# kyprifog/ballista

Measured on AMD Instinct MI355X. Metric: tpch_q1_sf100_rows_per_sec, higher is better.
Workload: dtype f64; 1 GPU; TPC-H Q1 SF100 (scan+filter+group-by aggregate), 600037902 lineitem rows resident in HBM, Arrow layout, Int32 order keys; lineitem_rows=600037902, rows_per_gpu=600037902, partitioning=1 GPU, whole tables

## Files before the change

### ballista_amd/_lib.py

```python
from __future__ import annotations

import ctypes as C
import os

_HERE = os.path.dirname(os.path.abspath(__file__))
LIB_PATH = os.environ.get("BHIP_LIB_PATH") or os.path.join(_HERE, "lib", "libballista_hip.so")

OK, EINVAL, ENOTIMPL, EEXEC, EHIP, EOOM = 0, 1, 2, 3, 4, 5


class BallistaError(Exception):

    def __init__(self, code, message):
        super().__init__(message)
        self.code = code


class NotImplementedOnGpu(BallistaError):
    """BHIP_ENOTIMPL — DataFusionError::NotImplemented: keep the CPU operator for this subtree."""


class PlanError(BallistaError):
    """BHIP_EINVAL — DataFusionError::Plan / Internal."""

# ... 73 lines not shown
class TpchOpts(C.Structure):
    _fields_ = [("key64", C.c_int32), ("with_dates", C.c_int32), ("sparse_keys", C.c_int32), ("n_columns", C.c_int32),
                ("key_base", C.c_int64), ("columns", C.POINTER(C.c_char_p))]


LEAF_RESOLVER = C.CFUNCTYPE(C.c_int32, C.c_void_p, C.POINTER(LeafDesc), C.POINTER(C.c_void_p))


class SortExprC(C.Structure):
    _fields_ = [("expr", Expr), ("descending", C.c_int32), ("nulls_first", C.c_int32)]


class WindowExprC(C.Structure):
    _fields_ = [("fn", C.c_int32), ("arg", Expr), ("offset", C.c_int64), ("frame", C.c_int32), ("name", C.c_char_p)]


class RowsFrameC(C.Structure):
    _fields_ = [("start_unbounded", C.c_int32), ("end_unbounded", C.c_int32), ("start", C.c_int64), ("end", C.c_int64)]


_P = C.c_void_p
_PP = C.POINTER(C.c_void_p)
SYMBOLS = {
    "bhip_last_error": (C.c_char_p, []),
    "bhip_version": (C.c_char_p, []),
    "bhip_ctx_create": (C.c_int32, [C.c_int, _PP]),
    "bhip_ctx_release": (None, [_P]),
    "bhip_ctx_synchronize": (C.c_int32, [_P]),
    "bhip_ctx_memory": (C.c_int32, [_P, C.POINTER(C.c_uint64), C.POINTER(C.c_uint64)]),
    "bhip_ctx_kernel_time": (C.c_int32, [_P, C.c_int32, C.POINTER(C.c_double), C.POINTER(C.c_uint64)]),
    "bhip_ctx_kernel_name": (C.c_char_p, [_P]),
    "bhip_ctx_kernel_variant": (C.c_char_p, [_P]),
    "bhip_ctx_lean_key_form": (C.c_char_p, [_P]),
    "bhip_ctx_sort_limit_form": (C.c_char_p, [_P]),
    "bhip_ctx_join_key_form": (C.c_char_p, [_P]),
    "bhip_ctx_nested_loop_form": (C.c_char_p, [_P]),
    "bhip_ctx_join_probe_form": (C.c_char_p, [_P]),
    "bhip_ctx_device_cus": (C.c_int32, [_P]),
    "bhip_ctx_kernel_stats": (C.c_int32, [_P, C.c_int32, C.c_char_p, C.c_size_t]),
    "bhip_batch_from_host": (C.c_int32, [_P, C.c_int32, C.POINTER(ColumnDesc), C.c_int64, _PP]),
    "bhip_batch_from_device": (C.c_int32, [_P, C.c_int32, C.POINTER(ColumnDesc), C.c_int64, _PP]),
    "bhip_batch_from_tbl": (C.c_int32, [_P, _P, C.c_int64, C.c_int32, C.POINTER(ColumnDesc), C.c_int32, C.POINTER(C.c_int32), _PP]),
    "bhip_batch_from_csv": (C.c_int32, [_P, _P, C.c_int64, C.c_int32, C.POINTER(ColumnDesc), C.c_int32, C.POINTER(C.c_int32),
                                        C.POINTER(CsvOpts), _PP]),
    "bhip_batch_import_arrow": (C.c_int32, [_P, _P, _P, _PP]),
    "bhip_batch_export_arrow": (C.c_int32, [_P, _P, _P]),
    "bhip_batch_retain": (None, [_P]),
    "bhip_batch_release": (None, [_P]),
    "bhip_batch_num_rows": (C.c_int64, [_P]),
    "bhip_batch_num_columns": (C.c_int32, [_P]),
    "bhip_batch_column_info": (C.c_int32, [_P, C.c_int32, C.POINTER(C.c_char_p), C.POINTER(C.c_int32),
                                           C.POINTER(C.c_int32), C.POINTER(C.c_int64), C.POINTER(C.c_int32)]),
    "bhip_batch_column_device": (C.c_int32, [_P, C.c_int32, _PP, _PP, _PP]),
    "bhip_batch_column_to_host": (C.c_int32, [_P, C.c_int32, _P, _P, _P]),
    "bhip_batch_memory_size": (C.c_int64, [_P]),
    "bhip_plan_memory": (C.c_int32, [_P, C.c_int32, C.POINTER(C.c_int32), _PP, _PP]),
    "bhip_plan_arrow_stream": (C.c_int32, [_P, _P, _PP]),
    "bhip_plan_arrow_streams": (C.c_int32, [_P, C.c_int32, _PP, _PP]),
    "bhip_plan_parquet": (C.c_int32, [_P, C.c_int32, C.POINTER(C.c_char_p), C.c_int32, C.POINTER(C.c_uint32), C.c_int32, _PP]),
    "bhip_plan_text_scan": (C.c_int32, [_P, C.c_int32, C.POINTER(C.c_char_p), C.c_int32, C.POINTER(ColumnDesc), C.c_int32,
                                        C.POINTER(C.c_int32), C.POINTER(TextScanOpts), _PP]),
    "bhip_plan_empty": (C.c_int32, [_P, C.c_int32, C.POINTER(ColumnDesc), C.c_int32, _PP]),
    "bhip_plan_filter": (C.c_int32, [_P, C.POINTER(Expr), _PP]),
    "bhip_plan_projection": (C.c_int32, [_P, C.c_int32, C.POINTER(Expr), C.POINTER(C.c_char_p), _PP]),
    "bhip_plan_hash_aggregate": (C.c_int32, [_P, C.c_int32, C.c_int32, C.POINTER(Expr), C.POINTER(C.c_char_p),
                                             C.c_int32, C.POINTER(Aggregate), _PP]),
# ... 81 lines not shown
```

### ballista_amd/csrc/host/capi.cpp

```cpp
#include <cstdio>
#include <cstring>

#include "../util_kernels.h"
#include "plan.hpp"

using namespace bhip;

#define BHIP_API_BEGIN try {
#define BHIP_API_END                                              \
    return BHIP_OK;                                               \
    }                                                             \
    catch (const bhip::Error& e) {                                \
        bhip::set_last_error(e.what());                           \
        return e.code;                                            \
    }                                                             \
    catch (const std::bad_alloc&) {                               \
        bhip::set_last_error("host allocation failed");           \
        return BHIP_EOOM;                                         \
    }                                                             \
    catch (const std::exception& e) {                             \
        bhip::set_last_error(std::string("internal error: ") + e.what()); \
        return BHIP_EINVAL;                                       \
    }                                                             \
    catch (...) {                                                 \
// ... 50 lines not shown
    need(ctx, "ctx"); need(buf, "buf");
    ctx->p->set_device();
    std::string text;
    for (auto& kv : ctx->p->kernel_stats(reset != 0)) {
        char line[256];
        snprintf(line, sizeof line, "%s\t%.6f\t%llu\t%llu\n", kv.first.c_str(), kv.second.ms, (unsigned long long)kv.second.launches,
                 (unsigned long long)kv.second.bytes);
        text += line;
    }
    if (text.size() + 1 > cap) fail(BHIP_EINVAL, "bhip_ctx_kernel_stats: buffer too small");
    memcpy(buf, text.c_str(), text.size() + 1);
    BHIP_API_END
}

const char* bhip_ctx_kernel_name(bhip_ctx* ctx) {
    static thread_local std::string name;
    name = ctx ? ctx->p->kernel_name() : std::string();
    return name.c_str();
}

int32_t bhip_ctx_device_cus(bhip_ctx* ctx) {
    return ctx ? ctx->p->cus() : 0;
}

const char* bhip_ctx_kernel_variant(bhip_ctx* ctx) {
    static thread_local std::string name;
    name = ctx ? ctx->p->kernel_variant() : std::string();
    return name.c_str();
}

const char* bhip_ctx_lean_key_form(bhip_ctx* ctx) {
    static thread_local std::string name;
    name = ctx ? ctx->p->lean_key_form() : std::string();
    return name.c_str();
}

const char* bhip_ctx_sort_limit_form(bhip_ctx* ctx) {
    static thread_local std::string name;
    name = ctx ? ctx->p->sort_limit_form() : std::string();
    return name.c_str();
}

const char* bhip_ctx_join_key_form(bhip_ctx* ctx) {
    static thread_local std::string name;
    name = ctx ? ctx->p->join_key_form() : std::string();
    return name.c_str();
}

const char* bhip_ctx_nested_loop_form(bhip_ctx* ctx) {
    static thread_local std::string name;
    name = ctx ? ctx->p->nested_loop_form() : std::string();
    return name.c_str();
}

const char* bhip_ctx_join_probe_form(bhip_ctx* ctx) {
    static thread_local std::string name;
    name = ctx ? ctx->p->join_probe_form() : std::string();
    return name.c_str();
}

static bhip_batch* wrap_batch(BatchPtr b) {
    auto h = new bhip_batch();
    h->p = std::move(b);
    return h;
}

// ... 654 lines not shown
```

### ballista_amd/csrc/host/core.cpp

```cpp
#include "core.hpp"

#include <immintrin.h>

#include <chrono>
#include <cstdlib>

#include "../util_kernels.h"

__attribute__((constructor)) static void bhip_runtime_defaults() { setenv("HIP_FORCE_DEV_KERNARG", "1", 0); }

namespace bhip {

static thread_local std::string t_last_error;
void set_last_error(const std::string& m) { t_last_error = m; }
const char* get_last_error() { return t_last_error.c_str(); }

const char* dtype_name(int dt) {
    switch (dt) {
        case DT_INT32: return "Int32";
        case DT_INT64: return "Int64";
        case DT_UINT8: return "UInt8";
        case DT_UINT64: return "UInt64";
        case DT_FLOAT64: return "Float64";
        case DT_DATE32: return "Date32";
// ... 251 lines not shown
        if (hipEventSynchronize(p.b) == hipSuccess && hipEventElapsedTime(&t, p.a, p.b) == hipSuccess) {
            auto& st = k_stats_[p.name];
            st.ms += t;
            st.launches += 1;
            st.bytes += p.bytes;
        }
        event_pool_.push_back(p.a);
        event_pool_.push_back(p.b);
    }
    pending_timed_.clear();
    auto out = k_stats_;
    if (reset) k_stats_.clear();
    return out;
}

std::string Context::kernel_name() {
    std::lock_guard<std::mutex> g(mu_);
    return k_name_;
}

std::string Context::kernel_variant() {
    std::lock_guard<std::mutex> g(mu_);
    return k_variant_;
}

void Context::set_lean_key_form(const char* form) {
    std::lock_guard<std::mutex> g(mu_);
    k_key_form_ = form ? form : "";
}

std::string Context::lean_key_form() {
    std::lock_guard<std::mutex> g(mu_);
    return k_key_form_;
}

void Context::set_sort_limit_form(const char* form) {
    std::lock_guard<std::mutex> g(mu_);
    k_sort_limit_form_ = form ? form : "";
}

std::string Context::sort_limit_form() {
    std::lock_guard<std::mutex> g(mu_);
    return k_sort_limit_form_;
}

void Context::set_join_key_form(const char* form) {
    std::lock_guard<std::mutex> g(mu_);
    k_join_key_form_ = form ? form : "";
}

std::string Context::join_key_form() {
    std::lock_guard<std::mutex> g(mu_);
    return k_join_key_form_;
}

void Context::set_nested_loop_form(const char* form) {
    std::lock_guard<std::mutex> g(mu_);
    k_nested_loop_form_ = form ? form : "";
}

std::string Context::nested_loop_form() {
    std::lock_guard<std::mutex> g(mu_);
    return k_nested_loop_form_;
}

void Context::set_join_probe_form(const char* form) {
// ... 189 lines not shown
```

### ballista_amd/csrc/host/core.hpp

```cpp
#pragma once
#include <hip/hip_runtime.h>
#include <atomic>
#include <cstdint>
#include <cstring>
#include <map>
#include <memory>
#include <mutex>
#include <stdexcept>
#include <string>
#include <vector>

#include "../../../include/ballista_hip.h"
#include "../kernels.h"

namespace bhip {

struct Error : std::runtime_error {
    bhip_status code;
    Error(bhip_status c, const std::string& m) : std::runtime_error(m), code(c) {}
};
[[noreturn]] inline void fail(bhip_status c, const std::string& m) { throw Error(c, m); }
inline void hip_check(hipError_t e, const char* what) {
    if (e != hipSuccess) {
        if (e == hipErrorOutOfMemory) fail(BHIP_EOOM, std::string(what) + ": " + hipGetErrorString(e));
// ... 10 lines not shown

class Context;

struct Block {
    void* ptr = nullptr;
    size_t bytes = 0;
    hipStream_t last_stream = nullptr;
    hipEvent_t ready = nullptr;
};

class Context : public std::enable_shared_from_this<Context> {
public:
    explicit Context(int device);
    ~Context();
    int device() const { return device_; }
    int cus() const { return cus_; }
    void set_device() const { HIP_CHECK(hipSetDevice(device_)); }

    void* alloc(size_t bytes, hipStream_t stream);
    void free(void* ptr, hipStream_t stream);
    void memory(uint64_t* in_use, uint64_t* peak);
    void trim();

    hipStream_t acquire_stream();
    void release_stream(hipStream_t s);

    void wait_stream(hipStream_t stream, const void* dev_src = nullptr, void* host_dst = nullptr, size_t bytes = 0);

    void add_kernel_time(double ms, uint64_t launches, const char* kernel = nullptr, const char* variant = nullptr);
    std::string kernel_name();
    std::string kernel_variant();
    void set_lean_key_form(const char* form);
    std::string lean_key_form();
    void set_sort_limit_form(const char* form);
    std::string sort_limit_form();
    void set_join_key_form(const char* form);
    std::string join_key_form();
    void set_nested_loop_form(const char* form);
    std::string nested_loop_form();
    void set_join_probe_form(const char* form);
    std::string join_probe_form();
    void kernel_time(bool reset, double* ms, uint64_t* launches);
    bool timing_enabled() const { return timing_ > 0; }
    int timing_level() const { return timing_; }
    struct KernelStat { double ms = 0; uint64_t launches = 0; uint64_t bytes = 0; };
    void push_timed(hipEvent_t a, hipEvent_t b, const char* name, uint64_t bytes = 0);
    hipEvent_t timing_event();
    std::map<std::string, KernelStat> kernel_stats(bool reset);

private:
    int device_;
    int cus_ = 256;
    int timing_ = 0;
    std::mutex mu_;
    std::multimap<size_t, Block> free_blocks_;
    std::map<void*, Block> live_;
    uint64_t in_use_ = 0, peak_ = 0, cached_ = 0;
    std::vector<hipStream_t> stream_pool_;
    static constexpr size_t N_SLOTS = 1024;
    struct HostSlot { volatile uint64_t w[8]; };
    HostSlot* slots_ = nullptr;
    std::atomic<uint64_t> slot_seq_{0};
    bool spin_wait_ = true;
    double k_ms_ = 0;
    uint64_t k_launches_ = 0;
    std::string k_name_, k_variant_, k_key_form_, k_sort_limit_form_, k_join_key_form_, k_nested_loop_form_, k_join_probe_form_;
    struct PendingTimed { hipEvent_t a, b; const char* name; uint64_t bytes; };
    std::vector<PendingTimed> pending_timed_;
    std::vector<hipEvent_t> event_pool_;
    std::map<std::string, KernelStat> k_stats_;
};
using ContextPtr = std::shared_ptr<Context>;

struct Exec {
    ContextPtr ctx;
    hipStream_t stream;
    LaunchCfg cfg() const { return LaunchCfg{ctx->cus(), stream}; }
};

struct KernelTimer {
    const Exec& ex;
    const char* name;
    hipEvent_t a = nullptr, b = nullptr;
    uint64_t bytes = 0;
    KernelTimer(const Exec& e, const char* n, int64_t rows = -1, uint64_t algorithmic_bytes = 0) : ex(e), name(n), bytes(algorithmic_bytes) {
        const int level = ex.ctx->timing_level();
        if (level <= 0 || (level == 1 && rows < (1 << 18))) return;
        a = ex.ctx->timing_event();
        b = ex.ctx->timing_event();
        hipEventRecord(a, ex.stream);
    }
    void stop() {
        if (!a) return;
        hipEventRecord(b, ex.stream);
        ex.ctx->push_timed(a, b, name, bytes);
        a = b = nullptr;
    }
    ~KernelTimer() { stop(); }
};
// ... 168 lines not shown
```

### ballista_amd/csrc/host/ops_agg.cpp

```cpp
#include "../sort_kernels.h"
#include "../util_kernels.h"
#include "hash_kernels.h"
#include "plan.hpp"
#include "sop.hpp"

namespace bhip {

static int sum_type(int t) {
    if (dt_is_float(t)) return t;
    if (dt_is_unsigned(t)) return DT_UINT64;
    return DT_INT64;
}

static int minmax_kind(int t, bool is_min) {
    if (dt_is_float(t)) return is_min ? ACC_MIN_F64 : ACC_MAX_F64;
    if (dt_is_unsigned(t)) return is_min ? ACC_MIN_U64 : ACC_MAX_U64;
    return is_min ? ACC_MIN_I64 : ACC_MAX_I64;
}

static const char* lowcard_launch_name(int gmax, bool batches) {
    if (batches) return gmax == 1 ? "scan_agg_lowcard_g1_batches" : gmax == 4 ? "scan_agg_lowcard_g4_batches" : "scan_agg_lowcard_g8_batches";
    return gmax == 1 ? "scan_agg_lowcard_g1" : gmax == 4 ? "scan_agg_lowcard_g4" : "scan_agg_lowcard_g8";
}

// ... 477 lines not shown
        HIP_CHECK(hipMemsetAsync(status, 0, sizeof(ScanStatus), ex.stream));
        int n_part = 0;
        const bool lean_now = use_lean && (gmax == 1 || gmax == 4);
        const bool sop_now = !lean_now && use_sop;
        key_layout = lean_now || sop_now ? &sop.key_info : &pb.key_info();
        int64_t cur_rows = 0;
        for (auto& b : cur) cur_rows += b->n_rows;
        const bool together = !lean_now && !sop_now && cur.size() > 1 && cur.size() <= 4096 && cur_rows <= (1 << 20);
        bool lens_seen = lean_now && !sampling;
        std::vector<ScanParams> Ps;
        if (together) {
            Ps.assign(cur.size(), P0);
            for (size_t i = 0; i < cur.size(); ++i) ProgramBuilder::bind(Ps[i], pb.columns(), *cur[i], nullable);
            int grid = 0;
            TIMED_LAUNCH(ex, lowcard_launch_name(gmax, true),
                         launch_scan_agg_lowcard(cfg, Ps[0], tmp.get<ScanParams>(cur.size()), gmax, partials, partial_ng, max_grid, status, &grid, (int)cur.size()));
            n_part = grid;
        }
        for (auto& b : cur) {
            if (together) break;
            ScanParams P = P0;
            ProgramBuilder::bind(P, pb.columns(), *b, nullable);
            int grid = 0;
            const bool timed = b->n_rows >= (1 << 16) || ((lean_now || sop_now) && ex.ctx->timing_level() >= 2);
            if (timed) {
                timer.begin();
                timer.kernel = lean_now ? "scan_agg_lean_kernel" : sop_now ? "scan_agg_sop_kernel" : "scan_agg_lowcard_kernel";
                timer.variant = nullptr;
            }
            if (lean_now) {
                bind_sop(sop, *b);
                const char* variant = nullptr;
                bool fixed_keys = false;
                HIP_CHECK(launch_scan_agg_lean(cfg, sop.prog, tmp.get<SopProgram>(1), gmax, partials + (size_t)n_part * gmax,
                                               partial_ng + n_part, max_grid, status, &grid, &variant, &fixed_keys));
                if (timed) timer.variant = variant;
                bool utf8_key = false;
                for (int q = 0; q < sop.prog.n_keys; ++q) utf8_key = utf8_key || sop.prog.keys[q].kind == SOP_KEY_UTF8;
                ex.ctx->set_lean_key_form(fixed_keys ? "fixed" : utf8_key ? "offsets" : "none");
                lens_seen = lens_seen && !fixed_keys;
            } else if (sop_now) {
                bind_sop(sop, *b);
                HIP_CHECK(launch_scan_agg_sop(cfg, sop.prog, tmp.get<SopProgram>(1), gmax, partials + (size_t)n_part * gmax,
                                              partial_ng + n_part, max_grid, status, &grid));
            } else
                TIMED_LAUNCH(ex, lowcard_launch_name(gmax, false),
                             launch_scan_agg_lowcard(cfg, P, tmp.get<ScanParams>(1), gmax, partials + (size_t)n_part * gmax,
                                                     partial_ng + n_part, max_grid, status, &grid));
            if (timed) timer.end();
            n_part += grid;
        }
        const int cap = 1024;
        table = tmp.get<GroupRec>(cap);
        uint32_t* entry_group = tmp.get<uint32_t>((size_t)n_part * gmax);
        AccSpec specs[VM_MAX_ACC];
        for (int i = 0; i < n_acc; ++i) specs[i] = P0.acc[i];
        TIMED_LAUNCH(ex, "merge_partials", launch_merge_partials(cfg, partials, partial_ng, n_part, gmax, specs, n_acc, table, cap, entry_group, status));
        early = EmitColumns();
        if (!sampling && !no_early_emit && group_.size() <= (size_t)TAIL_TOTALS) early = emit_table(table, cap, status, *key_layout);
        trace_point("aggregate: scan + merge + emit queued");
        tail = read_device(ex, info);
        const ScanStatus st = tail.st;
        timer.collect();
        if (lean_now && (st.flags & SCAN_ERR_KEY_TOO_LONG)) {
            use_lean = false;
            continue;
        }
        if (sop_now && (st.flags & SCAN_ERR_KEY_TOO_LONG)) {
            use_sop = false;
            continue;
        }
        check_scan_flags(st);
// ... 68 lines not shown
```

### ballista_amd/csrc/kernels_lean_spec.hip

```cpp
#include <stdlib.h>
#include "lean_spec_kernel.h"

namespace bhip {

hipError_t launch_scan_agg_lean_spec(const LaunchCfg& cfg, const SopProgram& S, SopProgram* dprog, int gmax, GroupRec* partials,
                                     uint32_t* partial_ng, int max_grid, ScanStatus* status, int* grid_out, bool* ran,
                                     const char** variant, bool* fixed) {
    static const bool no_fixed = env_flag("BHIP_NO_FIXED_UTF8");
#define BHIP_LEAN_SPEC(NAME_, GMAX_, NR_, R32_, K0_, K1_, NS_)                                                            \
    if (gmax == GMAX_ && !(no_fixed && (K0_ == LK_UTF8_FIXED || K1_ == LK_UTF8_FIXED)) &&                                 \
        lean_shape_matches<NR_, R32_, K0_, K1_, NS_>(S)) {                                                                \
        *ran = true;                                                                                                      \
        *variant = NAME_;                                                                                                 \
        *fixed = K0_ == LK_UTF8_FIXED || K1_ == LK_UTF8_FIXED;                                                            \
        return launch_sop_program(scan_agg_lean_spec_kernel<GMAX_, NR_, R32_, K0_, K1_, NS_>, LEAN_TILE, cfg, S, dprog,   \
                                  partials, partial_ng, max_grid, status, grid_out);                                      \
    }
    BHIP_LEAN_SPEC("lean_spec_q1", 4, 1, 0b1, LK_UTF8_FIXED, LK_UTF8_FIXED, 5)
    BHIP_LEAN_SPEC("lean_spec_q1", 4, 1, 0b1, LK_UTF8, LK_UTF8, 5)
    BHIP_LEAN_SPEC("lean_spec_key1", 4, 1, 0b1, LK_UTF8_FIXED, LK_NONE, 5)
    BHIP_LEAN_SPEC("lean_spec_key1", 4, 1, 0b1, LK_UTF8, LK_NONE, 5)
#undef BHIP_LEAN_SPEC
    *ran = false;
    return hipSuccess;
}

}
```

### ballista_amd/csrc/kernels_sop.hip

```cpp
#include <hip/hip_runtime.h>
#include <stdlib.h>
#include "sop.h"

namespace bhip {

hipError_t launch_scan_agg_sop_g1(const LaunchCfg&, const SopProgram&, SopProgram*, GroupRec*, uint32_t*, int, ScanStatus*, int*);
hipError_t launch_scan_agg_sop_g4(const LaunchCfg&, const SopProgram&, SopProgram*, GroupRec*, uint32_t*, int, ScanStatus*, int*);
hipError_t launch_scan_agg_sop_g8(const LaunchCfg&, const SopProgram&, SopProgram*, GroupRec*, uint32_t*, int, ScanStatus*, int*);

hipError_t launch_scan_agg_sop(const LaunchCfg& cfg, const SopProgram& S, SopProgram* dprog, int gmax, GroupRec* partials,
                               uint32_t* partial_ng, int max_grid, ScanStatus* status, int* grid_out) {
    switch (gmax) {
        case 1: return launch_scan_agg_sop_g1(cfg, S, dprog, partials, partial_ng, max_grid, status, grid_out);
        case 4: return launch_scan_agg_sop_g4(cfg, S, dprog, partials, partial_ng, max_grid, status, grid_out);
        case 8: return launch_scan_agg_sop_g8(cfg, S, dprog, partials, partial_ng, max_grid, status, grid_out);
        default: return hipErrorInvalidValue;
    }
}

hipError_t launch_scan_agg_lean_g1(const LaunchCfg&, const SopProgram&, SopProgram*, GroupRec*, uint32_t*, int, ScanStatus*, int*);
hipError_t launch_scan_agg_lean_g4(const LaunchCfg&, const SopProgram&, SopProgram*, GroupRec*, uint32_t*, int, ScanStatus*, int*);
hipError_t launch_scan_agg_lean_spec(const LaunchCfg&, const SopProgram&, SopProgram*, int, GroupRec*, uint32_t*, int, ScanStatus*, int*,
                                     bool*, const char**, bool*);

hipError_t launch_scan_agg_lean(const LaunchCfg& cfg, const SopProgram& S, SopProgram* dprog, int gmax, GroupRec* partials,
                                uint32_t* partial_ng, int max_grid, ScanStatus* status, int* grid_out, const char** variant,
                                bool* fixed_keys) {
    static const bool generic_only = env_flag("BHIP_LEAN_GENERIC");
    const char* name = "lean_generic";
    bool fixed = false;
    if (!variant) variant = &name;
    if (!fixed_keys) fixed_keys = &fixed;
    *fixed_keys = false;
    if (!generic_only) {
        bool ran = false;
        const hipError_t e = launch_scan_agg_lean_spec(cfg, S, dprog, gmax, partials, partial_ng, max_grid, status, grid_out, &ran, variant, fixed_keys);
        if (ran || e != hipSuccess) return e;
    }
    *variant = "lean_generic";
    switch (gmax) {
        case 1: return launch_scan_agg_lean_g1(cfg, S, dprog, partials, partial_ng, max_grid, status, grid_out);
        case 4: return launch_scan_agg_lean_g4(cfg, S, dprog, partials, partial_ng, max_grid, status, grid_out);
        default: return hipErrorInvalidValue;
    }
}

}
```

### ballista_amd/csrc/lean_spec_kernel.h

```cpp
#pragma once
#include "lean_kernel.h"

namespace bhip {

enum LeanKeyKind : int { LK_NONE = 0, LK_I32 = 1, LK_UTF8 = 2, LK_UTF8_FIXED = 3 };

template <int GMAX, int NR, int R32, int K0, int K1, int NS>
__global__ void __launch_bounds__(BLOCK, (GMAX == 1 && NS <= 5) ? 4 : 3)
scan_agg_lean_spec_kernel(const SopProgram* __restrict__ Sp, GroupRec* partials, uint32_t* partial_ng, ScanStatus* status) {
    static_assert(NR >= 1 && NR <= SOP_NRANGE && NS >= 1 && NS <= SOP_NSTEP && (K0 != LK_NONE || K1 == LK_NONE), "lean shape");
    const SopProgram& S = *Sp;
    constexpr int U = LEAN_U;
    constexpr int NKEY = 2;
    constexpr int KK[NKEY] = {K0, K1};
    constexpr bool HAS_OFFSETS = K0 == LK_UTF8 || K1 == LK_UTF8;
    constexpr bool HAS_FIXED = K0 == LK_UTF8_FIXED || K1 == LK_UTF8_FIXED;
    static_assert(!(HAS_OFFSETS && HAS_FIXED), "no mixed key forms: one unknown width sends the plan to the offsets form");
    __shared__ LeanLds<GMAX, NS> lds;
    const int tid = threadIdx.x, lane = tid & 63;

    const int64_t n_rows = S.n_rows;
    const int64_t n_tiles = n_rows / LEAN_TILE;
    const int64_t grid = gridDim.x;
    const int64_t my_tiles = (int64_t)blockIdx.x < n_tiles ? (n_tiles - 1 - (int64_t)blockIdx.x) / grid + 1 : 0;

    const BHIP_GLOBAL char* rbase[NR];
    double rlo[NR], rhi[NR];
#pragma unroll
    for (int p = 0; p < NR; ++p) {
        rbase[p] = (const BHIP_GLOBAL char*)S.cols[S.ranges[p].col].data;
        rlo[p] = S.ranges[p].lo; rhi[p] = S.ranges[p].hi;
    }
    const BHIP_GLOBAL char* kbase[NKEY];
    const BHIP_GLOBAL char* kdat[NKEY];
    uint32_t kw[NKEY];
#pragma unroll
    for (int q = 0; q < NKEY; ++q) {
        kbase[q] = nullptr; kdat[q] = nullptr; kw[q] = 0;
        if (KK[q] != LK_NONE) {
            const SopColumn c = S.cols[S.keys[q].col];
            kbase[q] = KK[q] == LK_UTF8 ? (const BHIP_GLOBAL char*)c.offsets : (const BHIP_GLOBAL char*)c.data;
            kdat[q] = (const BHIP_GLOBAL char*)c.data;
            if (KK[q] == LK_UTF8_FIXED) {
// ... 49 lines not shown
        }
    };
    auto add_row = [&](int lgr) {
        if constexpr (GMAX == 1) {
            rows1 += lgr >= 0 ? 1u : 0u;
        } else {
            const int g = lgr >= 0 ? lgr : 0;
            __hip_atomic_fetch_add(&lds.cnt[g * BLOCK + tid], lgr >= 0 ? 1u : 0u, __ATOMIC_RELAXED, __HIP_MEMORY_SCOPE_WORKGROUP);
        }
    };

    LeanU4 rv[NR][U];
    uint32_t kv[NKEY][U][2];
    uint64_t kb[NKEY][U];
    LeanU3 ko[2][NKEY][U];
    LeanU4 xv[NS][U];
#pragma unroll
    for (int u = 0; u < U; ++u) {
#pragma unroll
        for (int p = 0; p < NR; ++p) rv[p][u] = LeanU4{0, 0, 0, 0};
#pragma unroll
        for (int q = 0; q < NKEY; ++q) {
            kv[q][u][0] = kv[q][u][1] = 0; kb[q][u] = 0;
            ko[0][q][u] = ko[1][q][u] = LeanU3{0, 0, 0};
        }
    }
    const uint32_t t8 = (uint32_t)tid * 8u, t16 = (uint32_t)tid * 16u;
    uint32_t t2w[NKEY];
#pragma unroll
    for (int q = 0; q < NKEY; ++q) t2w[q] = (uint32_t)tid * 2u * kw[q];

    auto load_step = [&](int s, int64_t row) {
#pragma unroll
        for (int u = 0; u < U; ++u) xv[s][u] = lean_ld4(xbase[s] + (row + u * LEAN_SUB) * 8 + t16);
    };
    auto load_ranges = [&](int64_t row) {
#pragma unroll
        for (int p = 0; p < NR; ++p) {
            if ((R32 >> p) & 1) {
#pragma unroll
                for (int u = 0; u < U; ++u) {
                    const LeanU2 v = lean_ld2(rbase[p] + (row + u * LEAN_SUB) * 4 + t8);
                    rv[p][u].x = v.x; rv[p][u].y = v.y;
                }
            } else {
#pragma unroll
                for (int u = 0; u < U; ++u) rv[p][u] = lean_ld4(rbase[p] + (row + u * LEAN_SUB) * 8 + t16);
            }
        }
    };
    auto load_int_keys = [&](int64_t row) {
#pragma unroll
        for (int q = 0; q < NKEY; ++q)
            if (KK[q] == LK_I32) {
#pragma unroll
                for (int u = 0; u < U; ++u) {
                    const LeanU2 v = lean_ld2(kbase[q] + (row + u * LEAN_SUB) * 4 + t8);
                    kv[q][u][0] = v.x; kv[q][u][1] = v.y;
                }
            }
    };
    auto load_offsets = [&](LeanU3 (&o)[NKEY][U], int64_t row) {
#pragma unroll
        for (int q = 0; q < NKEY; ++q)
            if (KK[q] == LK_UTF8) {
#pragma unroll
                for (int u = 0; u < U; ++u) {
                    const BHIP_GLOBAL char* a = kbase[q] + (row + u * LEAN_SUB) * 4 + t8;
                    const LeanU2 v = lean_ld2(a);
                    o[q][u].a = v.x; o[q][u].b = v.y;
                    o[q][u].c = *(const BHIP_GLOBAL uint32_t*)(a + 8);
                }
            }
    };
    auto load_key_bytes = [&](const LeanU3 (&o)[NKEY][U]) {
#pragma unroll
        for (int q = 0; q < NKEY; ++q)
            if (KK[q] == LK_UTF8) {
#pragma unroll
                for (int u = 0; u < U; ++u) {
                    const uint32_t l0 = o[q][u].b - o[q][u].a, l1 = o[q][u].c - o[q][u].b;
                    lens.see(q, l0); lens.see(q, l1);
                    kv[q][u][0] = l0; kv[q][u][1] = l1;
                    kb[q][u] = ((const BHIP_GLOBAL PackedU64*)(kdat[q] + o[q][u].a))->v;
                }
            }
    };

    auto load_key_bytes_fixed = [&](int64_t row) {
#pragma unroll
// ... 43 lines not shown
                }
            } else if (KK[q] == LK_UTF8_FIXED) {
#pragma unroll
                for (int u = 0; u < U; ++u) {
                    w[q][2 * u] = lean_str_word((uint32_t)kb[q][u], kw[q]);
                    w[q][2 * u + 1] = lean_str_word((uint32_t)(kb[q][u] >> (kw[q] << 3)), kw[q]);
                }
            } else if (KK[q] == LK_I32) {
#pragma unroll
                for (int u = 0; u < U; ++u) { w[q][2 * u] = kv[q][u][0]; w[q][2 * u + 1] = kv[q][u][1]; }
            }
        }
#pragma unroll
        for (int r = 0; r < LEAN_ROWS; ++r) key[r] = ((uint64_t)w[1][r] << 32) | w[0][r];
    };
    auto tile = [&](auto P_, auto NEXT_, int64_t k) -> bool {
        constexpr int P = decltype(P_)::value;
        constexpr bool NEXT = decltype(NEXT_)::value;
        const int64_t row1 = tile_row(k + 1);
        bool live[LEAN_ROWS];
        uint64_t key[LEAN_ROWS];
        eval_live(live);
        eval_keys(key);
        if constexpr (NEXT) {
            load_ranges(row1);
            load_int_keys(row1);
            load_key_bytes(ko[P ^ 1]);
            load_key_bytes_fixed(row1);
            if constexpr (HAS_OFFSETS) load_offsets(ko[P], tile_row(k + 2));
        }
        int lg[LEAN_ROWS];
        if (!lookup(key, live, lg)) return false;
        double tp[LEAN_ROWS];
#pragma unroll
        for (int s = 0; s < NS; ++s) {
            double tv[LEAN_ROWS];
#pragma unroll
            for (int u = 0; u < U; ++u) {
                const LeanU4 x = xv[s][u];
                double a = u2d(((uint64_t)x.y << 32) | x.x), b = u2d(((uint64_t)x.w << 32) | x.z);
                if (!xplain[s]) {
                    a = u2d(((uint64_t)(x.y ^ xflip[s]) << 32) | x.x) + xadd[s];
                    b = u2d(((uint64_t)(x.w ^ xflip[s]) << 32) | x.z) + xadd[s];
                }
                tv[2 * u] = a; tv[2 * u + 1] = b;
            }
            if (s > 0 && !xstart[s]) {
#pragma unroll
                for (int r = 0; r < LEAN_ROWS; ++r) tv[r] = tp[r] * tv[r];
            }
#pragma unroll
            for (int r = 0; r < LEAN_ROWS; ++r) { add_step(lg[r], s, tv[r]); tp[r] = tv[r]; }
            if constexpr (NEXT) load_step(s, row1);
        }
#pragma unroll
        for (int r = 0; r < LEAN_ROWS; ++r) add_row(lg[r]);
        return true;
    };
    using I0 = std::integral_constant<int, 0>;
    using I1 = std::integral_constant<int, 1>;
    using BT = std::integral_constant<bool, true>;
    using BF = std::integral_constant<bool, false>;

    bool over = false;
    if (my_tiles > 0) {
        const int64_t row0 = tile_row(0);
        if constexpr (HAS_OFFSETS) load_offsets(ko[0], row0);
        load_key_bytes(ko[0]);
        load_key_bytes_fixed(row0);
        load_ranges(row0);
        load_int_keys(row0);
        if constexpr (HAS_OFFSETS) load_offsets(ko[1], tile_row(1));
#pragma unroll
        for (int s = 0; s < NS; ++s) load_step(s, row0);
        __builtin_amdgcn_s_waitcnt(0x0F70);
        int64_t k = 0;
        for (; k + 2 < my_tiles; k += 2) {
            if (!tile(I0{}, BT{}, k) || !tile(I1{}, BT{}, k + 1)) { over = true; break; }
        }
        if (!over) {
            if (my_tiles - k == 2) over = !tile(I0{}, BT{}, k) || !tile(I1{}, BF{}, k + 1);
            else over = !tile(I0{}, BF{}, k);
        }
    }

    if (!over && (int64_t)blockIdx.x == n_tiles % grid && n_tiles * LEAN_TILE < n_rows) {
        auto accumulate = [&](int lgr, const double (&tv)[NS]) {
#pragma unroll
            for (int s = 0; s < NS; ++s) add_step(lgr, s, tv[s]);
            add_row(lgr);
        };
        LeanLens<(GMAX > 1)> tail_lens;
        over = !lean_tail<GMAX, NS, NR>(S, n_tiles * LEAN_TILE, n_rows, HAS_FIXED ? tail_lens : lens, lookup, accumulate);
    }
    lean_finish<GMAX, NS>(lds, S, acc, rows1, lens, partials, partial_ng, status);
}

template <int NR, int R32, int K0, int K1, int NS>
static bool lean_shape_matches(const SopProgram& S) {
    if (S.n_ranges != NR || S.n_steps != NS) return false;
    for (int p = 0; p < NR; ++p) {
        if ((S.ranges[p].is32 != 0) != (((R32 >> p) & 1) != 0)) return false;
        if (S.cols[S.ranges[p].col].validity) return false;
    }
    const int kk[2] = {K0, K1};
    int n_keys = 0;
    for (int q = 0; q < 2; ++q) {
        if (kk[q] == LK_NONE) continue;
        ++n_keys;
        if (S.n_keys <= q) return false;
        if (S.keys[q].kind != (kk[q] == LK_I32 ? SOP_KEY_I32 : SOP_KEY_UTF8)) return false;
        const int32_t w = S.cols[S.keys[q].col].width;
        if (kk[q] == LK_UTF8_FIXED && (w < 1 || w > (int32_t)LEAN_MAX_STR)) return false;
    }
    return S.n_keys == n_keys;
}

}
```

### ballista_amd/csrc/sop.h

```cpp
#pragma once
#include <hip/hip_runtime.h>
#include <stdint.h>
#include "kernels.h"

namespace bhip {

constexpr int SOP_NRANGE = 4;
constexpr int SOP_NKEY = 3;
constexpr int SOP_NSTEP = 8;
constexpr int SOP_NCOL = 16;

struct SopColumn {
    const void* data;
    const int32_t* offsets;
    const uint64_t* validity;
    int32_t dtype;
    int32_t data_bytes;
    int32_t width;
    int32_t pad;
};

struct SopRange {
    uint8_t col;
    uint8_t is32;
// ... 2 lines not shown
};

struct SopStep {
    uint8_t col;
    uint8_t is32;
    uint8_t has_col;
    uint8_t start;
    uint8_t acc;
    uint8_t pad[3];
    double sgn, add;
};

enum SopKeyKind : uint8_t { SOP_KEY_I32 = 0, SOP_KEY_I64 = 1, SOP_KEY_UTF8 = 2 };
struct SopKey {
    uint8_t col;
    uint8_t kind;
    uint8_t pad[2];
};

struct SopProgram {
    int64_t n_rows;
    int32_t n_cols, n_ranges, n_keys, n_steps;
    SopColumn cols[SOP_NCOL];
    SopRange ranges[SOP_NRANGE];
    SopKey keys[SOP_NKEY];
    SopStep steps[SOP_NSTEP];
};

hipError_t launch_scan_agg_sop(const LaunchCfg& cfg, const SopProgram& S, SopProgram* dprog, int gmax, GroupRec* partials,
                               uint32_t* partial_ng, int max_grid, ScanStatus* status, int* grid_out);

hipError_t launch_scan_agg_lean(const LaunchCfg& cfg, const SopProgram& S, SopProgram* dprog, int gmax, GroupRec* partials,
                                uint32_t* partial_ng, int max_grid, ScanStatus* status, int* grid_out, const char** variant = nullptr,
                                bool* fixed_keys = nullptr);

hipError_t launch_range_bitmap(const LaunchCfg& cfg, const SopProgram& S, SopProgram* dprog, uint64_t* bitmap, uint32_t* tile_counts);
struct Utf8Literal { uint8_t bytes[64]; int32_t len; };
hipError_t launch_utf8_eq_bitmap(const LaunchCfg& cfg, const int32_t* offsets, const void* data, const uint64_t* validity, int64_t n, const Utf8Literal& lit,
                                 bool negate, uint64_t* bitmap, uint32_t* tile_counts);

}
```

### ballista_amd/plan.py

```python
from __future__ import annotations

import ctypes as C
import os
from typing import Iterator, List, Optional, Sequence, Tuple

import numpy as np

from . import _lib as L
from . import expr as E

DTYPE_ID = {E.INT32: 1, E.INT64: 2, E.UINT8: 3, E.UINT64: 4, E.FLOAT64: 5, E.DATE32: 6, E.BOOLEAN: 7, E.UTF8: 8,
            "Int8": 9, "Int16": 10, "UInt16": 11, "UInt32": 12, "Float32": 13, "Date64": 14, "Timestamp(Second)": 15,
            "Timestamp(Millisecond)": 16, "Timestamp(Microsecond)": 17, "Timestamp(Nanosecond)": 18,
            "LargeUtf8": 19, "Binary": 20}
DTYPE_NAME = {v: k for k, v in DTYPE_ID.items()}
NP_DTYPE = {E.INT32: np.int32, E.INT64: np.int64, E.UINT8: np.uint8, E.UINT64: np.uint64,
            E.FLOAT64: np.float64, E.DATE32: np.int32, E.INT8: np.int8, E.INT16: np.int16, E.UINT16: np.uint16,
            E.UINT32: np.uint32, E.FLOAT32: np.float32, E.DATE64: np.int64, E.TIMESTAMP_S: np.int64,
            E.TIMESTAMP_MS: np.int64, E.TIMESTAMP_US: np.int64, E.TIMESTAMP_NS: np.int64}

PARTIAL, FINAL = "Partial", "Final"
SINGLE = "Single"
INNER, LEFT, RIGHT = "Inner", "Left", "Right"
FULL, SEMI, ANTI, RIGHT_SEMI, RIGHT_ANTI = "Full", "Semi", "Anti", "RightSemi", "RightAnti"
# ... 18 lines not shown
        return {0: "UnknownPartitioning", 1: "RoundRobinBatch", 2: "Hash"}[self.scheme] + f"({self.count})"


class Context:

    def __init__(self, device: int = 0):
        h = C.c_void_p()
        L.check(L.lib().bhip_ctx_create(device, C.byref(h)))
        self._h = h

    def synchronize(self):
        L.check(L.lib().bhip_ctx_synchronize(self._h))

    def memory(self):
        a, b = C.c_uint64(), C.c_uint64()
        L.check(L.lib().bhip_ctx_memory(self._h, C.byref(a), C.byref(b)))
        return a.value, b.value

    def kernel_time(self, reset=False):
        ms, n = C.c_double(), C.c_uint64()
        L.check(L.lib().bhip_ctx_kernel_time(self._h, 1 if reset else 0, C.byref(ms), C.byref(n)))
        return ms.value, n.value

    def kernel_name(self, variant=False):
        name = L.lib().bhip_ctx_kernel_name(self._h).decode()
        if variant:
            v = L.lib().bhip_ctx_kernel_variant(self._h).decode()
            if v:
                name += "/" + v
        return name

    def lean_key_form(self):
        return L.lib().bhip_ctx_lean_key_form(self._h).decode()

    def sort_limit_form(self):
        return L.lib().bhip_ctx_sort_limit_form(self._h).decode()

    def join_key_form(self):
        return L.lib().bhip_ctx_join_key_form(self._h).decode()

    def join_probe_form(self):
        return L.lib().bhip_ctx_join_probe_form(self._h).decode()

    def nested_loop_form(self):
        return L.lib().bhip_ctx_nested_loop_form(self._h).decode()

    def device_cus(self):
        return int(L.lib().bhip_ctx_device_cus(self._h))

    def kernel_stats(self, reset=False):
        buf = C.create_string_buffer(1 << 16)
        L.check(L.lib().bhip_ctx_kernel_stats(self._h, 1 if reset else 0, buf, len(buf)))
        out = {}
        for line in buf.value.decode().splitlines():
            name, ms, n, nbytes = line.split("\t")
            out[name] = (float(ms), int(n), int(nbytes))
        return out

    def __del__(self):
        try:
            if getattr(self, "_h", None):
                L.lib().bhip_ctx_release(self._h)
                self._h = None
        except Exception:
            pass

# ... 1018 lines not shown
```

### include/ballista_hip.h

```cpp
#ifndef BALLISTA_HIP_H
#define BALLISTA_HIP_H

#include <stddef.h>
#include <stdint.h>

#ifdef __cplusplus
extern "C" {
#endif

#ifndef ARROW_C_DATA_INTERFACE
#define ARROW_C_DATA_INTERFACE
#define ARROW_FLAG_DICTIONARY_ORDERED 1
#define ARROW_FLAG_NULLABLE 2
#define ARROW_FLAG_MAP_KEYS_SORTED 4
struct ArrowSchema {
    const char* format;
    const char* name;
    const char* metadata;
    int64_t flags;
    int64_t n_children;
    struct ArrowSchema** children;
    struct ArrowSchema* dictionary;
    void (*release)(struct ArrowSchema*);
    void* private_data;
// ... 294 lines not shown
    uint64_t rows_in, rows_out, chunks, streamed;
    uint64_t bytes_sent_remote, bytes_kept_local, staging_bytes;
    uint64_t rows_to[BHIP_SHUFFLE_MAX_PEERS];
    double ms_count, ms_total;
} bhip_shuffle_stats;
bhip_status bhip_comm_shuffle(bhip_comm* comm, bhip_batch* batch, const char* key_column, int64_t chunk_rows, bhip_batch** out,
                              bhip_shuffle_stats* stats);
bhip_status bhip_plan_all_gather(bhip_comm* comm, bhip_plan* input, bhip_plan** out);
bhip_status bhip_plan_shuffle(bhip_comm* comm, bhip_plan* input, const char* key_column, int64_t chunk_rows, bhip_plan** out);
bhip_status bhip_batch_pack(bhip_batch* batch, int64_t* header, int32_t header_cap, void* host_block, int64_t block_cap,
                            int64_t* block_bytes);
bhip_status bhip_batch_unpack(bhip_ctx* ctx, int32_t n_cols, const bhip_column_desc* schema, const int64_t* header,
                              const void* host_block, bhip_batch** out);

bhip_status bhip_tpch_lineitem(bhip_ctx* ctx, double sf, uint64_t seed, uint64_t row0, uint64_t n, int32_t key64,
                               int32_t with_dates, bhip_batch** out);
bhip_status bhip_tpch_orders(bhip_ctx* ctx, double sf, uint64_t seed, uint64_t row0, uint64_t n, int32_t key64,
                             bhip_batch** out);
typedef struct bhip_tpch_opts {
    int32_t key64, with_dates, sparse_keys, n_columns;
    int64_t key_base;
    const char* const* columns;
} bhip_tpch_opts;
bhip_status bhip_tpch_lineitem_opts(bhip_ctx* ctx, double sf, uint64_t seed, uint64_t row0, uint64_t n, const bhip_tpch_opts* opts,
                                    bhip_batch** out);
bhip_status bhip_tpch_orders_opts(bhip_ctx* ctx, double sf, uint64_t seed, uint64_t row0, uint64_t n, const bhip_tpch_opts* opts,
                                  bhip_batch** out);

bhip_status bhip_ctx_kernel_time(bhip_ctx* ctx, int32_t reset, double* ms, uint64_t* launches);
bhip_status bhip_ctx_kernel_stats(bhip_ctx* ctx, int32_t reset, char* buf, size_t cap);
const char* bhip_ctx_kernel_name(bhip_ctx* ctx);
const char* bhip_ctx_kernel_variant(bhip_ctx* ctx);
const char* bhip_ctx_lean_key_form(bhip_ctx* ctx);
const char* bhip_ctx_sort_limit_form(bhip_ctx* ctx);
const char* bhip_ctx_join_key_form(bhip_ctx* ctx);
const char* bhip_ctx_nested_loop_form(bhip_ctx* ctx);
const char* bhip_ctx_join_probe_form(bhip_ctx* ctx);
int32_t bhip_ctx_device_cus(bhip_ctx* ctx);

#ifdef __cplusplus
}
#endif
#endif
```

Before: 157.7 billion rows/s.

## Alias repeated column loads in lean Q1 kernel and use nontemporal streaming loads

Detects aggregation steps that read the same input column (Q1's sum(l_quantity), avg(l_quantity) and similar repeats, alias pattern 0,1,2,3,2) and specializes the lean kernel so each distinct column is loaded once and its value reused for the aliased steps. Separately, the column, range and key loads switch to nontemporal loads so streamed data does not pollute the cache. This targets redundant HBM traffic in a bandwidth-bound scan. It doubles the number of template instantiations and adds a diagnostic API for reporting the alias map.

```diff
diff --git a/ballista_amd/_lib.py b/ballista_amd/_lib.py
--- a/ballista_amd/_lib.py
+++ b/ballista_amd/_lib.py
@@ -129,6 +129,7 @@
     "bhip_ctx_kernel_name": (C.c_char_p, [_P]),
     "bhip_ctx_kernel_variant": (C.c_char_p, [_P]),
     "bhip_ctx_lean_key_form": (C.c_char_p, [_P]),
+    "bhip_ctx_lean_step_alias": (C.c_char_p, [_P]),
     "bhip_ctx_sort_limit_form": (C.c_char_p, [_P]),
     "bhip_ctx_join_key_form": (C.c_char_p, [_P]),
     "bhip_ctx_nested_loop_form": (C.c_char_p, [_P]),
diff --git a/ballista_amd/csrc/host/capi.cpp b/ballista_amd/csrc/host/capi.cpp
--- a/ballista_amd/csrc/host/capi.cpp
+++ b/ballista_amd/csrc/host/capi.cpp
@@ -106,6 +106,12 @@
 const char* bhip_ctx_lean_key_form(bhip_ctx* ctx) {
     static thread_local std::string name;
     name = ctx ? ctx->p->lean_key_form() : std::string();
+    return name.c_str();
+}
+
+const char* bhip_ctx_lean_step_alias(bhip_ctx* ctx) {
+    static thread_local std::string name;
+    name = ctx ? ctx->p->lean_step_alias() : std::string();
     return name.c_str();
 }
 
diff --git a/ballista_amd/csrc/host/core.cpp b/ballista_amd/csrc/host/core.cpp
--- a/ballista_amd/csrc/host/core.cpp
+++ b/ballista_amd/csrc/host/core.cpp
@@ -307,6 +307,23 @@
 std::string Context::lean_key_form() {
     std::lock_guard<std::mutex> g(mu_);
     return k_key_form_;
+}
+
+void Context::set_lean_step_alias(uint32_t alias, int n_steps) {
+    std::string list;
+    bool aliased = false;
+    for (int s = 0; s < n_steps; ++s) {
+        const int a = (int)((alias >> (4 * s)) & 15u);
+        aliased = aliased || a != s;
+        list += (s ? "," : "") + std::to_string(a);
+    }
+    std::lock_guard<std::mutex> g(mu_);
+    k_step_alias_ = aliased ? list : "none";
+}
+
+std::string Context::lean_step_alias() {
+    std::lock_guard<std::mutex> g(mu_);
+    return k_step_alias_;
 }
 
 void Context::set_sort_limit_form(const char* form) {
diff --git a/ballista_amd/csrc/host/core.hpp b/ballista_amd/csrc/host/core.hpp
--- a/ballista_amd/csrc/host/core.hpp
+++ b/ballista_amd/csrc/host/core.hpp
@@ -66,6 +66,8 @@
     std::string kernel_variant();
     void set_lean_key_form(const char* form);
     std::string lean_key_form();
+    void set_lean_step_alias(uint32_t alias, int n_steps);
+    std::string lean_step_alias();
     void set_sort_limit_form(const char* form);
     std::string sort_limit_form();
     void set_join_key_form(const char* form);
@@ -98,7 +100,7 @@
     bool spin_wait_ = true;
     double k_ms_ = 0;
     uint64_t k_launches_ = 0;
-    std::string k_name_, k_variant_, k_key_form_, k_sort_limit_form_, k_join_key_form_, k_nested_loop_form_, k_join_probe_form_;
+    std::string k_name_, k_variant_, k_key_form_, k_step_alias_, k_sort_limit_form_, k_join_key_form_, k_nested_loop_form_, k_join_probe_form_;
     struct PendingTimed { hipEvent_t a, b; const char* name; uint64_t bytes; };
     std::vector<PendingTimed> pending_timed_;
     std::vector<hipEvent_t> event_pool_;
diff --git a/ballista_amd/csrc/host/ops_agg.cpp b/ballista_amd/csrc/host/ops_agg.cpp
--- a/ballista_amd/csrc/host/ops_agg.cpp
+++ b/ballista_amd/csrc/host/ops_agg.cpp
@@ -533,12 +533,14 @@
                 bind_sop(sop, *b);
                 const char* variant = nullptr;
                 bool fixed_keys = false;
+                uint32_t step_alias = 0;
                 HIP_CHECK(launch_scan_agg_lean(cfg, sop.prog, tmp.get<SopProgram>(1), gmax, partials + (size_t)n_part * gmax,
-                                               partial_ng + n_part, max_grid, status, &grid, &variant, &fixed_keys));
+                                               partial_ng + n_part, max_grid, status, &grid, &variant, &fixed_keys, &step_alias));
                 if (timed) timer.variant = variant;
                 bool utf8_key = false;
                 for (int q = 0; q < sop.prog.n_keys; ++q) utf8_key = utf8_key || sop.prog.keys[q].kind == SOP_KEY_UTF8;
                 ex.ctx->set_lean_key_form(fixed_keys ? "fixed" : utf8_key ? "offsets" : "none");
+                ex.ctx->set_lean_step_alias(step_alias, sop.prog.n_steps);
                 lens_seen = lens_seen && !fixed_keys;
             } else if (sop_now) {
                 bind_sop(sop, *b);
diff --git a/ballista_amd/csrc/kernels_lean_spec.hip b/ballista_amd/csrc/kernels_lean_spec.hip
--- a/ballista_amd/csrc/kernels_lean_spec.hip
+++ b/ballista_amd/csrc/kernels_lean_spec.hip
@@ -5,22 +5,30 @@
 
 hipError_t launch_scan_agg_lean_spec(const LaunchCfg& cfg, const SopProgram& S, SopProgram* dprog, int gmax, GroupRec* partials,
                                      uint32_t* partial_ng, int max_grid, ScanStatus* status, int* grid_out, bool* ran,
-                                     const char** variant, bool* fixed) {
+                                     const char** variant, bool* fixed, uint32_t* step_alias) {
     static const bool no_fixed = env_flag("BHIP_NO_FIXED_UTF8");
-#define BHIP_LEAN_SPEC(NAME_, GMAX_, NR_, R32_, K0_, K1_, NS_)                                                            \
+    static const bool no_alias = env_flag("BHIP_LEAN_NO_ALIAS");
+    const uint32_t alias = lean_step_alias(S);
+#define BHIP_LEAN_SPEC_A(NAME_, GMAX_, NR_, R32_, K0_, K1_, NS_, ALIAS_)                                                  \
     if (gmax == GMAX_ && !(no_fixed && (K0_ == LK_UTF8_FIXED || K1_ == LK_UTF8_FIXED)) &&                                 \
+        (ALIAS_ == lean_alias_identity(NS_) || (!no_alias && alias == ALIAS_)) &&                                         \
         lean_shape_matches<NR_, R32_, K0_, K1_, NS_>(S)) {                                                                \
         *ran = true;                                                                                                      \
         *variant = NAME_;                                                                                                 \
         *fixed = K0_ == LK_UTF8_FIXED || K1_ == LK_UTF8_FIXED;                                                            \
-        return launch_sop_program(scan_agg_lean_spec_kernel<GMAX_, NR_, R32_, K0_, K1_, NS_>, LEAN_TILE, cfg, S, dprog,   \
-                                  partials, partial_ng, max_grid, status, grid_out);                                      \
+        *step_alias = ALIAS_;                                                                                             \
+        return launch_sop_program(scan_agg_lean_spec_kernel<GMAX_, NR_, R32_, K0_, K1_, NS_, ALIAS_>, LEAN_TILE, cfg, S,  \
+                                  dprog, partials, partial_ng, max_grid, status, grid_out);                               \
     }
+#define BHIP_LEAN_SPEC(NAME_, GMAX_, NR_, R32_, K0_, K1_, NS_)                                                            \
+    BHIP_LEAN_SPEC_A(NAME_, GMAX_, NR_, R32_, K0_, K1_, NS_, 0x23210u)                                                    \
+    BHIP_LEAN_SPEC_A(NAME_, GMAX_, NR_, R32_, K0_, K1_, NS_, lean_alias_identity(NS_))
     BHIP_LEAN_SPEC("lean_spec_q1", 4, 1, 0b1, LK_UTF8_FIXED, LK_UTF8_FIXED, 5)
     BHIP_LEAN_SPEC("lean_spec_q1", 4, 1, 0b1, LK_UTF8, LK_UTF8, 5)
     BHIP_LEAN_SPEC("lean_spec_key1", 4, 1, 0b1, LK_UTF8_FIXED, LK_NONE, 5)
     BHIP_LEAN_SPEC("lean_spec_key1", 4, 1, 0b1, LK_UTF8, LK_NONE, 5)
 #undef BHIP_LEAN_SPEC
+#undef BHIP_LEAN_SPEC_A
     *ran = false;
     return hipSuccess;
 }
diff --git a/ballista_amd/csrc/kernels_sop.hip b/ballista_amd/csrc/kernels_sop.hip
--- a/ballista_amd/csrc/kernels_sop.hip
+++ b/ballista_amd/csrc/kernels_sop.hip
@@ -21,23 +21,27 @@
 hipError_t launch_scan_agg_lean_g1(const LaunchCfg&, const SopProgram&, SopProgram*, GroupRec*, uint32_t*, int, ScanStatus*, int*);
 hipError_t launch_scan_agg_lean_g4(const LaunchCfg&, const SopProgram&, SopProgram*, GroupRec*, uint32_t*, int, ScanStatus*, int*);
 hipError_t launch_scan_agg_lean_spec(const LaunchCfg&, const SopProgram&, SopProgram*, int, GroupRec*, uint32_t*, int, ScanStatus*, int*,
-                                     bool*, const char**, bool*);
+                                     bool*, const char**, bool*, uint32_t*);
 
 hipError_t launch_scan_agg_lean(const LaunchCfg& cfg, const SopProgram& S, SopProgram* dprog, int gmax, GroupRec* partials,
                                 uint32_t* partial_ng, int max_grid, ScanStatus* status, int* grid_out, const char** variant,
-                                bool* fixed_keys) {
+                                bool* fixed_keys, uint32_t* step_alias) {
     static const bool generic_only = env_flag("BHIP_LEAN_GENERIC");
     const char* name = "lean_generic";
     bool fixed = false;
+    uint32_t alias = 0;
     if (!variant) variant = &name;
     if (!fixed_keys) fixed_keys = &fixed;
+    if (!step_alias) step_alias = &alias;
     *fixed_keys = false;
     if (!generic_only) {
         bool ran = false;
-        const hipError_t e = launch_scan_agg_lean_spec(cfg, S, dprog, gmax, partials, partial_ng, max_grid, status, grid_out, &ran, variant, fixed_keys);
+        const hipError_t e = launch_scan_agg_lean_spec(cfg, S, dprog, gmax, partials, partial_ng, max_grid, status, grid_out, &ran, variant, fixed_keys, step_alias);
         if (ran || e != hipSuccess) return e;
     }
     *variant = "lean_generic";
+    *step_alias = 0;
+    for (int s = 0; s < S.n_steps; ++s) *step_alias |= (uint32_t)s << (4 * s);
     switch (gmax) {
         case 1: return launch_scan_agg_lean_g1(cfg, S, dprog, partials, partial_ng, max_grid, status, grid_out);
         case 4: return launch_scan_agg_lean_g4(cfg, S, dprog, partials, partial_ng, max_grid, status, grid_out);
diff --git a/ballista_amd/csrc/lean_spec_kernel.h b/ballista_amd/csrc/lean_spec_kernel.h
--- a/ballista_amd/csrc/lean_spec_kernel.h
+++ b/ballista_amd/csrc/lean_spec_kernel.h
@@ -5,10 +5,36 @@
 
 enum LeanKeyKind : int { LK_NONE = 0, LK_I32 = 1, LK_UTF8 = 2, LK_UTF8_FIXED = 3 };
 
-template <int GMAX, int NR, int R32, int K0, int K1, int NS>
+constexpr uint32_t lean_alias_of(uint32_t alias, int s) { return (alias >> (4 * s)) & 15u; }
+constexpr uint32_t lean_alias_identity(int ns) {
+    uint32_t a = 0;
+    for (int s = 0; s < ns; ++s) a |= (uint32_t)s << (4 * s);
+    return a;
+}
+constexpr bool lean_alias_valid(uint32_t alias, int ns) {
+    for (int s = 0; s < ns; ++s) {
+        const uint32_t a = lean_alias_of(alias, s);
+        if (a > (uint32_t)s || lean_alias_of(alias, (int)a) != a) return false;
+    }
+    return true;
+}
+
+typedef uint32_t LeanV2 __attribute__((ext_vector_type(2)));
+typedef uint32_t LeanV4 __attribute__((ext_vector_type(4)));
+__device__ inline LeanU2 lean_stream_ld2(const BHIP_GLOBAL char* p) {
+    const LeanV2 v = __builtin_nontemporal_load((const BHIP_GLOBAL LeanV2*)p);
+    return LeanU2{v.x, v.y};
+}
+__device__ inline LeanU4 lean_stream_ld4(const BHIP_GLOBAL char* p) {
+    const LeanV4 v = __builtin_nontemporal_load((const BHIP_GLOBAL LeanV4*)p);
+    return LeanU4{v.x, v.y, v.z, v.w};
+}
+
+template <int GMAX, int NR, int R32, int K0, int K1, int NS, uint32_t ALIAS = lean_alias_identity(NS)>
 __global__ void __launch_bounds__(BLOCK, (GMAX == 1 && NS <= 5) ? 4 : 3)
 scan_agg_lean_spec_kernel(const SopProgram* __restrict__ Sp, GroupRec* partials, uint32_t* partial_ng, ScanStatus* status) {
     static_assert(NR >= 1 && NR <= SOP_NRANGE && NS >= 1 && NS <= SOP_NSTEP && (K0 != LK_NONE || K1 == LK_NONE), "lean shape");
+    static_assert(lean_alias_valid(ALIAS, NS), "a(s) <= s and a(a(s)) == a(s)");
     const SopProgram& S = *Sp;
     constexpr int U = LEAN_U;
     constexpr int NKEY = 2;
@@ -124,7 +150,7 @@
 
     auto load_step = [&](int s, int64_t row) {
 #pragma unroll
-        for (int u = 0; u < U; ++u) xv[s][u] = lean_ld4(xbase[s] + (row + u * LEAN_SUB) * 8 + t16);
+        for (int u = 0; u < U; ++u) xv[s][u] = lean_stream_ld4(xbase[s] + (row + u * LEAN_SUB) * 8 + t16);
     };
     auto load_ranges = [&](int64_t row) {
 #pragma unroll
@@ -132,12 +158,12 @@
             if ((R32 >> p) & 1) {
 #pragma unroll
                 for (int u = 0; u < U; ++u) {
-                    const LeanU2 v = lean_ld2(rbase[p] + (row + u * LEAN_SUB) * 4 + t8);
+                    const LeanU2 v = lean_stream_ld2(rbase[p] + (row + u * LEAN_SUB) * 4 + t8);
                     rv[p][u].x = v.x; rv[p][u].y = v.y;
                 }
             } else {
 #pragma unroll
-                for (int u = 0; u < U; ++u) rv[p][u] = lean_ld4(rbase[p] + (row + u * LEAN_SUB) * 8 + t16);
+                for (int u = 0; u < U; ++u) rv[p][u] = lean_stream_ld4(rbase[p] + (row + u * LEAN_SUB) * 8 + t16);
             }
         }
     };
@@ -147,7 +173,7 @@
             if (KK[q] == LK_I32) {
 #pragma unroll
                 for (int u = 0; u < U; ++u) {
-                    const LeanU2 v = lean_ld2(kbase[q] + (row + u * LEAN_SUB) * 4 + t8);
+                    const LeanU2 v = lean_stream_ld2(kbase[q] + (row + u * LEAN_SUB) * 4 + t8);
                     kv[q][u][0] = v.x; kv[q][u][1] = v.y;
                 }
             }
@@ -257,18 +283,30 @@
         int lg[LEAN_ROWS];
         if (!lookup(key, live, lg)) return false;
         double tp[LEAN_ROWS];
+        double fa[NS][LEAN_ROWS];
+        auto factor = [&](int s, const LeanU4 x, double& a, double& b) {
+            a = u2d(((uint64_t)x.y << 32) | x.x); b = u2d(((uint64_t)x.w << 32) | x.z);
+            if (!xplain[s]) {
+                a = u2d(((uint64_t)(x.y ^ xflip[s]) << 32) | x.x) + xadd[s];
+                b = u2d(((uint64_t)(x.w ^ xflip[s]) << 32) | x.z) + xadd[s];
+            }
+        };
 #pragma unroll
         for (int s = 0; s < NS; ++s) {
+            const bool own = lean_alias_of(ALIAS, s) == (uint32_t)s;
             double tv[LEAN_ROWS];
-#pragma unroll
-            for (int u = 0; u < U; ++u) {
-                const LeanU4 x = xv[s][u];
-                double a = u2d(((uint64_t)x.y << 32) | x.x), b = u2d(((uint64_t)x.w << 32) | x.z);
-                if (!xplain[s]) {
-                    a = u2d(((uint64_t)(x.y ^ xflip[s]) << 32) | x.x) + xadd[s];
-                    b = u2d(((uint64_t)(x.w ^ xflip[s]) << 32) | x.z) + xadd[s];
-                }
-                tv[2 * u] = a; tv[2 * u + 1] = b;
+            if (own) {
+#pragma unroll
+                for (int u = 0; u < U; ++u) factor(s, xv[s][u], tv[2 * u], tv[2 * u + 1]);
+#pragma unroll
+                for (int a = s + 1; a < NS; ++a)
+                    if (lean_alias_of(ALIAS, a) == (uint32_t)s) {
+#pragma unroll
+                        for (int u = 0; u < U; ++u) factor(a, xv[s][u], fa[a][2 * u], fa[a][2 * u + 1]);
+                    }
+            } else {
+#pragma unroll
+                for (int r = 0; r < LEAN_ROWS; ++r) tv[r] = fa[s][r];
             }
             if (s > 0 && !xstart[s]) {
 #pragma unroll
@@ -276,7 +314,7 @@
             }
 #pragma unroll
             for (int r = 0; r < LEAN_ROWS; ++r) { add_step(lg[r], s, tv[r]); tp[r] = tv[r]; }
-            if constexpr (NEXT) load_step(s, row1);
+            if constexpr (NEXT) { if (own) load_step(s, row1); }
         }
 #pragma unroll
         for (int r = 0; r < LEAN_ROWS; ++r) add_row(lg[r]);
@@ -297,7 +335,8 @@
         load_int_keys(row0);
         if constexpr (HAS_OFFSETS) load_offsets(ko[1], tile_row(1));
 #pragma unroll
-        for (int s = 0; s < NS; ++s) load_step(s, row0);
+        for (int s = 0; s < NS; ++s)
+            if (lean_alias_of(ALIAS, s) == (uint32_t)s) load_step(s, row0);
         __builtin_amdgcn_s_waitcnt(0x0F70);
         int64_t k = 0;
         for (; k + 2 < my_tiles; k += 2) {
@@ -319,6 +358,17 @@
         over = !lean_tail<GMAX, NS, NR>(S, n_tiles * LEAN_TILE, n_rows, HAS_FIXED ? tail_lens : lens, lookup, accumulate);
     }
     lean_finish<GMAX, NS>(lds, S, acc, rows1, lens, partials, partial_ng, status);
+}
+
+static uint32_t lean_step_alias(const SopProgram& S) {
+    uint32_t alias = 0;
+    for (int s = 0; s < S.n_steps && s < SOP_NSTEP; ++s) {
+        int a = s;
+        for (int e = s - 1; e >= 0; --e)
+            if (S.steps[e].col == S.steps[s].col && S.steps[e].is32 == S.steps[s].is32) a = e;
+        alias |= (uint32_t)a << (4 * s);
+    }
+    return alias;
 }
 
 template <int NR, int R32, int K0, int K1, int NS>
diff --git a/ballista_amd/csrc/sop.h b/ballista_amd/csrc/sop.h
--- a/ballista_amd/csrc/sop.h
+++ b/ballista_amd/csrc/sop.h
@@ -58,7 +58,7 @@
 
 hipError_t launch_scan_agg_lean(const LaunchCfg& cfg, const SopProgram& S, SopProgram* dprog, int gmax, GroupRec* partials,
                                 uint32_t* partial_ng, int max_grid, ScanStatus* status, int* grid_out, const char** variant = nullptr,
-                                bool* fixed_keys = nullptr);
+                                bool* fixed_keys = nullptr, uint32_t* step_alias = nullptr);
 
 hipError_t launch_range_bitmap(const LaunchCfg& cfg, const SopProgram& S, SopProgram* dprog, uint64_t* bitmap, uint32_t* tile_counts);
 struct Utf8Literal { uint8_t bytes[64]; int32_t len; };
diff --git a/ballista_amd/plan.py b/ballista_amd/plan.py
--- a/ballista_amd/plan.py
+++ b/ballista_amd/plan.py
@@ -74,6 +74,9 @@
 
     def lean_key_form(self):
         return L.lib().bhip_ctx_lean_key_form(self._h).decode()
+
+    def lean_step_alias(self):
+        return L.lib().bhip_ctx_lean_step_alias(self._h).decode()
 
     def sort_limit_form(self):
         return L.lib().bhip_ctx_sort_limit_form(self._h).decode()
diff --git a/include/ballista_hip.h b/include/ballista_hip.h
--- a/include/ballista_hip.h
+++ b/include/ballista_hip.h
@@ -350,6 +350,7 @@
 const char* bhip_ctx_kernel_name(bhip_ctx* ctx);
 const char* bhip_ctx_kernel_variant(bhip_ctx* ctx);
 const char* bhip_ctx_lean_key_form(bhip_ctx* ctx);
+const char* bhip_ctx_lean_step_alias(bhip_ctx* ctx);
 const char* bhip_ctx_sort_limit_form(bhip_ctx* ctx);
 const char* bhip_ctx_join_key_form(bhip_ctx* ctx);
 const char* bhip_ctx_nested_loop_form(bhip_ctx* ctx);
```

New measurement: 172.8 billion rows/s (median of 6 runs). 9.5% higher.
